# facebookresearch/ReAgent

Hardware: AMD Instinct MI355X
Metric: transitions/sec at batch=65536 state_dim=128; 1/2/4/8 MI355X scaling (higher is better)
Workload: dtype bf16; 1 GPU; Discrete DQN state_dim=128 |A|=16 3x512 MLP (BASELINE.json configs[1]; replay gather + normalize + 3 fwd + TD/Huber + bwd + Adam + soft update); batch=65536/GPU, 3x512 hidden; global_batch=65536, parallelism=dp1, launch=graph replay

## Files before the change

### profiles/microbench/fwd_phases.hip

```cpp
#include <hip/hip_runtime.h>
__device__ unsigned long long* g_stamps;
#define RG_STAMP(slot)                                                                                   \
  do {                                                                                                   \
    if ((threadIdx.x & 63) == 0)                                                                         \
      g_stamps[((long)blockIdx.x * (blockDim.x >> 6) + (threadIdx.x >> 6)) * 20 + (slot)] = __builtin_amdgcn_s_memtime(); \
  } while (0)
#include "../../reagent_amd/csrc/mlp_fused.hip"
namespace rg {
int x3_forward_launch(const rg_mlp_desc*, MlpArgs&, hipStream_t) { return RG_EINVAL; }
int x3_backward_launch(const rg_mlp_desc*, MlpArgs&, hipStream_t) { return RG_EINVAL; }
void grouped_bias_reduce_launch(const float*, const int*, int, int, float*, int, hipStream_t) {}
}
#include <cstdio>
#include <vector>

namespace rg {
template <int TN, int NW, int PITCH>
__global__ void RG_LAUNCH_BOUNDS(NW * 64, 1) fwd_some_save_kernel(MlpArgs saving, MlpArgs plain, int every) {
  if ((int)blockIdx.x & every) mlp_fwd_fused_body<TN, NW, PITCH, false>(saving);
  else mlp_fwd_fused_body<TN, NW, PITCH, false>(plain);
}
}

int main(int argc, char** argv) {
  using namespace rg;
  const int save = argc > 1 ? atoi(argv[1]) : 0;
  const int B = 65536, dims[5] = {128, 512, 512, 512, 16};
  MlpArgs a{};
  a.n_layers = 4; a.batch = B;
  for (int i = 0; i < 5; ++i) a.dims[i] = dims[i];
  for (int l = 0; l < 4; ++l) {
    a.acts[l] = l < 3 ? ACT_RELU : ACT_LINEAR;
    void* w; const size_t n = rg_wfrag_elems(dims[l + 1], dims[l]);
    hipMalloc(&w, n * 2); hipMemset(w, 0x3c, n * 2);
    a.wfrag[l] = (const bf16_t*)w;
    float* b; hipMalloc((void**)&b, dims[l + 1] * 4); hipMemset(b, 0, dims[l + 1] * 4);
    a.bias[l] = b;
    if (save) {
      void* f; hipMalloc(&f, rg_frag_elems(B, dims[l]) * 2); a.act_frag[l] = (bf16_t*)f;
      if (l >= 1) { void* sg; hipMalloc(&sg, rg_sign_bytes(B, dims[l])); a.act_sign[l] = (unsigned*)sg; }
    }
  }
  float *x, *out;
  hipMalloc((void**)&x, (size_t)B * 128 * 4); hipMemset(x, 0x3c, (size_t)B * 128 * 4);
  hipMalloc((void**)&out, (size_t)B * 16 * 4);
  a.x = x; a.ldx = 128; a.x_is_f32 = 1; a.out32 = out; a.ldo = 16; a.pitch = 520; a.save = save;
  const int n_wg = argc > 2 ? atoi(argv[2]) : B / 128, NPH = 20, NWV = FB_NW;
  unsigned long long* stamps;
  hipMalloc((void**)&stamps, (size_t)n_wg * NWV * NPH * 8);
  hipMemcpyToSymbol(HIP_SYMBOL(g_stamps), &stamps, sizeof(stamps));
  a.out_lds = argc > 3 ? atoi(argv[3]) : 0;
  const size_t lds = (size_t)128 * 520 * 2 + (a.out_lds ? 32 * 512 : 0);
  const int every = argc > 4 ? atoi(argv[4]) : 0;
  MlpArgs plain = a;
  plain.save = 0;
  hipFuncSetAttribute((const void*)mlp_fwd_fused_kernel<512 / (32 * FB_NW), FB_NW, 520>, hipFuncAttributeMaxDynamicSharedMemorySize, (int)lds);
  hipFuncSetAttribute((const void*)fwd_some_save_kernel<512 / (32 * FB_NW), FB_NW, 520>, hipFuncAttributeMaxDynamicSharedMemorySize, (int)lds);
  auto launch = [&] {
    if (every) fwd_some_save_kernel<512 / (32 * FB_NW), FB_NW, 520><<<n_wg, FB_NW * 64, lds>>>(a, plain, every);
    else mlp_fwd_fused_kernel<512 / (32 * FB_NW), FB_NW, 520><<<n_wg, FB_NW * 64, lds>>>(a);
  };
  hipEvent_t e0, e1; hipEventCreate(&e0); hipEventCreate(&e1);
  for (int w = 0; w < 3; ++w) launch();
  hipDeviceSynchronize();
  hipEventRecord(e0);
  for (int r = 0; r < 20; ++r) launch();
  hipEventRecord(e1); hipEventSynchronize(e1);
  float ms; hipEventElapsedTime(&ms, e0, e1);
  printf("forward NW=%d RING=%d save=%d: %.2f us/launch (stamps on), err=%d\n", FB_NW, MlpCfg<FB_NW>::RING, save, ms * 1e3 / 20, (int)hipGetLastError());
  std::vector<unsigned long long> h((size_t)n_wg * NWV * NPH);
  hipMemcpy(h.data(), stamps, h.size() * 8, hipMemcpyDeviceToHost);
  const char* names[NPH] = {"", "x tile load+barrier", "L0 mainloop(K=128)", "L0 pack", "L0 barrier wait", "L0 LDS store+barrier",
                            "L1 mainloop(K=512)", "L1 pack", "L1 barrier wait", "L1 LDS store+barrier",
                            "L2 mainloop(K=512)", "L2 pack", "L2 barrier wait", "L2 LDS store+barrier", "output layer", ""};
  double tot[NPH] = {0}, span = 0;
  int n_counted = 0;
  for (int g = 0; g < n_wg; ++g) {
    if (every && !(g & every)) continue;
    ++n_counted;
    for (int w = 0; w < NWV; ++w) {
      const unsigned long long* s = &h[((size_t)g * NWV + w) * NPH];
      for (int p = 1; p <= 14; ++p) tot[p] += (double)(s[p] - s[p - 1]);
      span += (double)(s[14] - s[0]);
    }
  }
  const double nw = (double)n_counted * NWV;
  if (every) printf("only workgroups with (index & %d) save: the tables below cover those %d\n", every, n_counted);
  printf("workgroups %d, shader clock %.3f GHz (ticks of one round / launch time)\n", n_wg, (span / nw) * ((n_wg + 255) / 256) / (ms * 1e6 / 20));
  printf("avg s_memtime ticks per wave: %.0f\n", span / nw);
  for (int p = 1; p <= 14; ++p) printf("  %-22s %9.0f ticks  %5.1f %%\n", names[p], tot[p] / nw, 100.0 * tot[p] / span);
  {
    double t[4] = {0, 0, 0, 0}, t19 = 0, n19 = 0;
    for (int g = 0; g < n_wg; ++g)
      for (int w = 0; w < NWV; ++w) {
        const unsigned long long* s = &h[((size_t)g * NWV + w) * NPH];
        if (!s[16] || (every && !(g & every))) continue;
        if (s[19]) { t19 += (double)(s[19] - s[18]); n19 += 1; }
        t[0] += (double)(s[16] - s[13]); t[1] += (double)(s[17] - s[16]); t[2] += (double)(s[18] - s[17]); t[3] += (double)(s[14] - s[18]);
      }
    printf("  storing waves: LDS sum %.0f ticks (of their sum + stores)\n", t19 / (n19 > 0 ? n19 : 1));
    printf("  output layer split: K loop %.0f | barrier wait %.0f | hand-off + barrier %.0f | sum + stores %.0f ticks\n", t[0] / nw, t[1] / nw, t[2] / nw, t[3] / nw);
  }
  printf("per-wave L1 main loop / barrier wait (ticks), averaged over workgroups:\n");
  for (int w = 0; w < NWV; ++w) {
    double ml = 0, bw = 0, ep = 0;
    for (int g = 0; g < n_wg; ++g) {
      const unsigned long long* s = &h[((size_t)g * NWV + w) * NPH];
      ml += (double)(s[6] - s[5]); bw += (double)(s[7] - s[6]); ep += (double)(s[8] - s[7]);
    }
    printf("  wave %d: mainloop %8.0f  pack %8.0f  wait %8.0f\n", w, ml / n_wg, bw / n_wg, ep / n_wg);
  }
  return 0;
}
```

### reagent_amd/csrc/mlp_fused.hip

```cpp

#include "rg_mlp_frag.h"
#include "rg_reduce.h"
#include "rg_dqn_head_row.h"

namespace rg {

constexpr int GROUPED_RING = 8;

template <int NW> struct MlpCfg {
  static constexpr int THREADS = NW * 64;
  static constexpr int RING = NW == 4 ? 8 : 2;
};

template <int NW>
__device__ __forceinline__ void grouped_whole_tile_out(bf16_t* act, int pitch, int KC, const bf16_t* wf_out, const float* b_out,
                                                                 int N, int NTo, int out_act, int lo, int hi, int row_base,
                                                                 const int* scatter, int batch, float* out32, long ldo) {
  const int tid = threadIdx.x, lane = tid & 63, wave = wave_uniform(tid >> 6), lr = lane & 31, lg = lane >> 5;
  const int P = NTo * 32 + 4, np = N >> 2;
  f32x16 acc4[4][1];
#pragma unroll
  for (int tm = 0; tm < 4; ++tm)
#pragma unroll
    for (int r = 0; r < 16; ++r) acc4[tm][0][r] = 0.f;
  const int col = wave * 32 + lr;
  float b = 0.f;
  if (wave < NTo) {
    if (b_out && col < N) b = b_out[col];
    wide_mainloop<1, GROUPED_RING>(act, pitch, KC, wf_out + (long)wave * KC * 512, 0, acc4, lane, k_rotation(blockIdx.x, wave, KC));
  }
  RG_STAMP(16);
  __syncthreads();
  RG_STAMP(17);
  float* stage = (float*)act;
  if (wave < NTo) {
#pragma unroll
    for (int tm = 0; tm < 4; ++tm) {
      float v[16];
#pragma unroll
      for (int r = 0; r < 16; ++r) v[r] = acc4[tm][0][r] + b;
      act_apply_n(v, out_act);
#pragma unroll
      for (int r = 0; r < 16; ++r) stage[(tm * 32 + (r & 3) + 8 * (r >> 2) + 4 * lg) * P + col] = v[r];
    }
  }
  __syncthreads();
  RG_STAMP(18);
  for (int rel = lo + wave; rel < hi; rel += NW) {
    int row = row_base + rel;
    if (scatter) row = scatter[row];
    if (row >= 0 && (scatter || row < batch) && lane < np)
      stream_store(*(const f32x4*)(stage + rel * P + lane * 4), (f32x4*)(out32 + (long)row * ldo + lane * 4));
  }
  RG_STAMP(19);
}

template <int TN, int NW, int PITCH, bool GROUPED, bool PAIR = false>
__device__ __forceinline__ void mlp_fwd_fused_body(const MlpArgs& a, const PairArgs* pp = nullptr, int pass = 0, bool on_state = false) {
  constexpr int THREADS = MlpCfg<NW>::THREADS, RING = MlpCfg<NW>::RING;
  static_assert(!PAIR || (!GROUPED && NW == 8), "the pair is the plain 8-wave kernel");
  const int save = PAIR ? (on_state ? 1 : 0) : a.save;
  RG_DYN_LDS(smem);
  bf16_t* act = (bf16_t*)smem;
  const int tid = PAIR ? opaque((int)threadIdx.x) : (int)threadIdx.x, lane = tid & 63, wave = wave_uniform(tid >> 6);
  const int lr = lane & 31, lg = lane >> 5;
  const int tile = GROUPED ? grouped_tile(blockIdx.x, (a.batch + FB_BM - 1) / FB_BM) : (int)blockIdx.x;
  if (GROUPED && tile * FB_BM >= round_up(a.batch, FB_BM)) return;
  const int row_base = tile * FB_BM;
  constexpr int pitch = PITCH;
  const int k0p = round_up(a.dims[0], 32);
  RG_STAMP(0);
  if constexpr (PAIR) {
    const PairIO& io = pp->io[on_state ? 1 : 0];
    const void* x = io.x;
    const long ldx = io.ldx;
    if (io.x_is_f32)
      load_tile_to_lds<float, THREADS>(act, pitch, (const float*)x, ldx, row_base, a.batch, a.dims[0], k0p, tid);
    else
      load_tile_to_lds<bf16_t, THREADS>(act, pitch, (const bf16_t*)x, ldx, row_base, a.batch, a.dims[0], k0p, tid);
  } else if (a.rowmap) {
    if (a.x_is_f32)
      load_tile_rows_mapped<float, THREADS>(act, pitch, (const float*)a.x, a.ldx, a.rowmap, row_base, a.dims[0], k0p, tid);
    else
      load_tile_rows_mapped<bf16_t, THREADS>(act, pitch, (const bf16_t*)a.x, a.ldx, a.rowmap, row_base, a.dims[0], k0p, tid);
  } else if (a.x2) {
    const int n2 = a.dims[0] - a.x_split;
    if (a.x_is_f32)
      load_tile_to_lds<float, THREADS>(act, pitch, (const float*)a.x, a.ldx, row_base, a.batch, a.x_split, a.x_split, tid, a.x_tile);
    else
      load_tile_to_lds<bf16_t, THREADS>(act, pitch, (const bf16_t*)a.x, a.ldx, row_base, a.batch, a.x_split, a.x_split, tid, a.x_tile);
    if (a.x2_is_f32)
      load_tile_to_lds<float, THREADS>(act + a.x_split, pitch, (const float*)a.x2, a.ldx2, row_base, a.batch, n2, k0p - a.x_split, tid);
    else
      load_tile_to_lds<bf16_t, THREADS>(act + a.x_split, pitch, (const bf16_t*)a.x2, a.ldx2, row_base, a.batch, n2, k0p - a.x_split, tid);
  } else if (a.x_is_f32)
    load_tile_to_lds<float, THREADS>(act, pitch, (const float*)a.x, a.ldx, row_base, a.batch, a.dims[0], k0p, tid);
  else
    load_tile_to_lds<bf16_t, THREADS>(act, pitch, (const bf16_t*)a.x, a.ldx, row_base, a.batch, a.dims[0], k0p, tid);
  __syncthreads();
  RG_STAMP(1);
  if (save == 1 && a.act_frag[0]) emit_frags_from_lds(act, pitch, k0p / 32, a.act_frag[0], tile * 4, wave, NW, lane);
  const bool out_lds = PAIR || (!GROUPED && a.out_lds);
  char* wo = (char*)(act + FB_BM * pitch);
  if (out_lds && pass == 0) out_lds_prefetch(a.wfrag[a.n_layers - 1], (a.dims[a.n_layers - 1] + 15) / 16, wo, wave, NW, lane);

  for (int l = 0; l < a.n_layers; ++l) {
    const int K = a.dims[l], N = a.dims[l + 1];
    const int KC = (K + 15) / 16;
    if (l < a.n_layers - 1) {
      f32x16 acc[4][TN];
#pragma unroll
      for (int tm = 0; tm < 4; ++tm)
#pragma unroll
        for (int tn = 0; tn < TN; ++tn)
#pragma unroll
          for (int r = 0; r < 16; ++r) acc[tm][tn][r] = 0.f;
      const long nt_stride = (long)KC * 512;
      wide_mainloop<TN, RING>(act, pitch, KC, a.wfrag[l] + (long)(wave * TN) * nt_stride, nt_stride, acc, lane,
                              k_rotation(blockIdx.x, wave, KC), wave / (NW / 2));
      RG_STAMP(2 + 4 * l);
      unsigned PK[4][TN][8];
      unsigned* sign_dst = save ? a.act_sign[l + 1] : nullptr;
      if constexpr (PAIR) {
        fwd_hidden_pack<TN, ACT_RELU>(acc, a.bias[l], save ? a.act_frag[l + 1] : nullptr, sign_dst, N / 32, tile * 4, wave, lane, PK);
      } else {
        RG_DISPATCH_ACT(a.acts[l], (fwd_hidden_pack<TN, A_>(acc, a.bias[l], fwd_save_dst(a, l),
                                                            sign_dst, N / 32, tile * 4, wave, lane, PK)));
      }
      RG_STAMP(3 + 4 * l);
      __syncthreads();
      RG_STAMP(4 + 4 * l);
      store_packed_tiles<TN>(act, pitch, PK, wave, lane);
      if (out_lds) RG_WAIT_VMCNT(0);
      __syncthreads();
      RG_STAMP(5 + 4 * l);
    } else {
      const int NTo = (N + 31) / 32;
      const int out_act = a.acts[l];
      const bool stream_out = N > 64;
      int seg_g = GROUPED ? a.tile_key[tile] : 0;
      RowSegment seg{0, 0, FB_BM};
      const int o_lane = GROUPED ? opaque(lane) : lane, o_tid = GROUPED ? opaque(tid) : tid;
      while (!GROUPED || next_segment(a.row_begin, a.n_groups, row_base, FB_BM, seg_g, seg)) {
        const int lane = o_lane, tid = o_tid, lr = lane & 31, lg = lane >> 5;
        const int grp = seg.grp;
        const bf16_t* wf_out = a.wfrag[l] + (GROUPED ? (long)grp * a.group_stride : 0);
        const float* b_out = a.bias[l] ? a.bias[l] + (GROUPED ? (long)grp * N : 0) : nullptr;
        const int tm0 = GROUPED ? seg.lo >> 5 : 0, tm1 = GROUPED ? (seg.hi + 31) >> 5 : 4;
        const float b_tile0 = (b_out && lr < N) ? b_out[lr] : 0.f;
        auto store_tile = [&](const f32x16& acc, int tm, int nt) {
          const int col = nt * 32 + lr;
          if (col < N) {
            const float b = nt == 0 ? b_tile0 : (b_out ? b_out[col] : 0.f);
            float ov[16];
#pragma unroll
            for (int r = 0; r < 16; ++r) ov[r] = acc[r] + b;
            act_apply_n(ov, out_act);
#pragma unroll
            for (int r = 0; r < 16; ++r) {
              const int rel = tm * 32 + (r & 3) + 8 * (r >> 2) + 4 * lg;
              if (GROUPED && (rel < seg.lo || rel >= seg.hi)) continue;
              int row = row_base + rel;
              if (a.out_scatter) row = a.rowmap[row];
              if (row >= 0 && (a.out_scatter || row < a.batch)) {
                const float o = ov[r];
                if (stream_out) stream_store(o, a.out32 + (long)row * a.ldo + col);
                else a.out32[(long)row * a.ldo + col] = o;
              }
            }
          }
        };
        f32x4 h_m4, h_qt4, h_ac4;
        float h_rew = 0.f, h_nt = 0.f, h_ge = 0.f;
        int h_b = 0;
        bool h_live = false;
        if constexpr (PAIR) {
          if (pass == 1) {
            const int it = wave * 64 + opaque(lane), row = row_base + (it >> 2);
            h_live = row < a.batch;
            h_b = h_live ? row : a.batch - 1;
            const long o = (long)h_b * 16 + (it & 3) * 4;
            h_m4 = *(const f32x4*)(pp->next_mask + o);
            h_qt4 = *(const f32x4*)(pp->qn_target + o);
            h_ac4 = *(const f32x4*)(pp->action + o);
            h_rew = pp->reward[h_b];
            h_nt = pp->not_terminal[h_b];
            if (pp->gamma_exponent) h_ge = pp->gamma_exponent[h_b];
          }
        }
        if (PAIR || (!GROUPED && NTo == 1 && NW == 8 && KC >= 8)) {
          const int tm = wave & 3, half = wave >> 2, kc_mid = (KC / 2 + 3) / 4 * 4;
          f32x16 acc = out_lds ? tile_kloop_ldsb(act, pitch, wo, tm, lane, half ? kc_mid : 0, half ? KC : kc_mid)
                               : tile_kloop(act, pitch, KC, wf_out, tm, 0, lane, half ? kc_mid : 0, half ? KC : kc_mid);
          RG_STAMP(16);
          __syncthreads();
          RG_STAMP(17);
          const int o_ln = opaque(lane), o_lr = o_ln & 31, o_lg = o_ln >> 5;
          const bool aligned16 = (reinterpret_cast<uintptr_t>(a.out32) & 15) == 0;
          const bool dense_run = a.ldo == N && row_base + FB_BM <= a.batch;
          const bool rowstore = PAIR || (!a.out_scatter && aligned16 && (dense_run || ((N & 3) == 0 && (a.ldo & 3) == 0)));
          if (rowstore) {
            float* outs = (float*)act + half * (FB_BM * 32);
            float* bias_s = (float*)act + 2 * (FB_BM * 32);
            if (o_lr < N) {
#pragma unroll
              for (int r = 0; r < 16; ++r) outs[(tm * 32 + (r & 3) + 8 * (r >> 2) + 4 * o_lg) * N + o_lr] = acc[r];
              if (wave == 0 && o_lg == 0) bias_s[o_lr] = b_tile0;
            }
            __syncthreads();
            RG_STAMP(18);
            RG_STAMP(19);
            const float* lo_ = (const float*)act;
            const float* hi_ = lo_ + FB_BM * 32;
            if constexpr (PAIR) {
              const int it = wave * 64 + o_ln, rel = it >> 2, c4 = it & 3, row = row_base + rel;
              const f32x4 l4 = *(const f32x4*)(lo_ + it * 4), h4 = *(const f32x4*)(hi_ + it * 4);
              const f32x4 b4 = *(const f32x4*)(bias_s + c4 * 4);
              float o[4];
#pragma unroll
              for (int e = 0; e < 4; ++e) o[e] = (l4[e] + h4[e]) + b4[e];
              act_apply_n(o, out_act);
              const f32x4 mine = f32x4{o[0], o[1], o[2], o[3]};
              if (row < a.batch) *(f32x4*)(pp->io[on_state ? 1 : 0].out + (long)row * 16 + c4 * 4) = mine;
              f32x4* park = (f32x4*)(wo + (size_t)KC * 512);
              if (pass == 0) {
                park[it] = mine;
              } else {
                const f32x4 other = park[it];
                const f32x4 q4 = on_state ? mine : other, qon4 = on_state ? other : mine;
                const float loss = dqn_head_lanes_row<4>(h_m4, h_qt4, pp->double_q ? qon4 : h_qt4, h_ac4, q4, c4, h_b, h_live, h_rew,
                                                         pp->reward_boosts, h_nt, pp->gamma, pp->gamma_exponent != nullptr, h_ge,
                                                         a.batch, pp->double_q, pp->loss_type, pp->dq, pp->next_q, pp->next_idx,
                                                         pp->q_sel);
                const float ws = dqn_head_wave_sum(loss);
                if (o_ln == 0) pp->wave_sums[tile * NW + wave] = ws;
              }
            } else if (dense_run) {
              float* dst = a.out32 + (long)row_base * N;
              for (int it = wave * 64 + o_ln; it < (FB_BM * N) >> 2; it += THREADS) {
                const f32x4 l4 = *(const f32x4*)(lo_ + it * 4), h4 = *(const f32x4*)(hi_ + it * 4);
                float o[4];
#pragma unroll
                for (int e = 0; e < 4; ++e) o[e] = (l4[e] + h4[e]) + bias_s[(it * 4 + e) % N];
                act_apply_n(o, out_act);
                *(f32x4*)(dst + it * 4) = f32x4{o[0], o[1], o[2], o[3]};
              }
            }
            const int np = N >> 2;
            for (int it = wave * 64 + o_ln; !PAIR && !dense_run && it < FB_BM * np; it += THREADS) {
              const int rel = it / np, c4 = it - rel * np;
              const int row = row_base + rel;
              if (row < a.batch) {
                const f32x4 l4 = *(const f32x4*)(lo_ + rel * N + c4 * 4), h4 = *(const f32x4*)(hi_ + rel * N + c4 * 4);
                const f32x4 b4 = *(const f32x4*)(bias_s + c4 * 4);
                float o[4];
#pragma unroll
                for (int e = 0; e < 4; ++e) o[e] = (l4[e] + h4[e]) + b4[e];
                act_apply_n(o, out_act);
                *(f32x4*)(a.out32 + (long)row * a.ldo + c4 * 4) = f32x4{o[0], o[1], o[2], o[3]};
              }
            }
          } else {
            float* hand = (float*)act + (tm * 64 + lane) * 16;
            if (half) {
#pragma unroll
              for (int r = 0; r < 16; r += 4) *(f32x4*)(hand + r) = f32x4{acc[r], acc[r + 1], acc[r + 2], acc[r + 3]};
            }
            __syncthreads();
            RG_STAMP(18);
            if (!half) {
#pragma unroll
              for (int r = 0; r < 16; r += 4) {
                const f32x4 o = *(const f32x4*)(hand + r);
                acc[r] += o[0]; acc[r + 1] += o[1]; acc[r + 2] += o[2]; acc[r + 3] += o[3];
              }
              RG_STAMP(19);
              store_tile(acc, tm, 0);
            }
          }
        } else if (GROUPED && NTo <= NW && a.stage_out) {
          const int P = NTo * 32 + 4;
          const int np = N >> 2;
          bool last_segment = false;
          if ((size_t)FB_BM * P * sizeof(float) <= (size_t)FB_BM * pitch * sizeof(bf16_t)) {
            int g2 = seg_g;
            RowSegment s2;
            last_segment = !next_segment(a.row_begin, a.n_groups, row_base, FB_BM, g2, s2);
          }
          if (last_segment) {
            grouped_whole_tile_out<NW>(act, pitch, KC, wf_out, b_out, N, NTo, out_act, seg.lo, seg.hi, row_base, a.out_scatter ? a.rowmap : nullptr,
                                       a.batch, a.out32, a.ldo);
            break;
          }
          float* stage = (float*)(act + FB_BM * pitch);
          for (int tm = tm0; tm < tm1; ++tm) {
            if (wave < NTo) {
              const f32x16 acc = tile_kloop(act, pitch, KC, wf_out, tm, wave, lane);
              const int col = wave * 32 + lr;
              const float b = (b_out && col < N) ? b_out[col] : 0.f;
              float v[16];
#pragma unroll
              for (int r = 0; r < 16; ++r) v[r] = acc[r] + b;
              act_apply_n(v, out_act);
#pragma unroll
              for (int r = 0; r < 16; ++r) stage[((r & 3) + 8 * (r >> 2) + 4 * lg) * P + col] = v[r];
            }
            __syncthreads();
            for (int it = tid; it < 32 * np; it += THREADS) {
              const int r = it / np, c4 = it - r * np;
              const int rel = tm * 32 + r;
              if (rel < seg.lo || rel >= seg.hi) continue;
              int row = row_base + rel;
              if (a.out_scatter) row = a.rowmap[row];
              if (row >= 0 && (a.out_scatter || row < a.batch))
                stream_store(*(const f32x4*)(stage + r * P + c4 * 4), (f32x4*)(a.out32 + (long)row * a.ldo + c4 * 4));
            }
            __syncthreads();
          }
        } else {
          for (int t = wave; t < 4 * NTo; t += NW) {
            const int tm = t & 3, nt = t >> 2;
            if (tm < tm0 || tm >= tm1) continue;
            store_tile(tile_kloop(act, pitch, KC, wf_out, tm, nt, lane), tm, nt);
          }
        }
        if (!GROUPED) break;
      }
      RG_STAMP(2 + 4 * l);
    }
  }
}

#ifndef RG_PAIR_ORDER_SHIFT
#define RG_PAIR_ORDER_SHIFT 0
#endif
template <int TN, int NW, int PITCH>
__global__ void RG_LAUNCH_BOUNDS(NW * 64, 1) mlp_fwd_pair_kernel(MlpArgs a, PairArgs p) {
  const bool state_first = (((int)blockIdx.x >> RG_PAIR_ORDER_SHIFT) & 1) != 0;
  mlp_fwd_fused_body<TN, NW, PITCH, false, true>(a, &p, 0, state_first);
  __syncthreads();
  mlp_fwd_fused_body<TN, NW, PITCH, false, true>(a, &p, 1, !state_first);
}

template <int TN, int NW, int PITCH>
__global__ void RG_LAUNCH_BOUNDS(NW * 64, 1) mlp_fwd_fused_kernel(MlpArgs a) {
  mlp_fwd_fused_body<TN, NW, PITCH, false>(a);
}
template <int TN, int NW, int PITCH>
__global__ void RG_LAUNCH_BOUNDS(NW * 64, 1) mlp_fwd_grouped_kernel(MlpArgs a) {
  mlp_fwd_fused_body<TN, NW, PITCH, true>(a);
}

template <int TN, int NW, int PITCH, bool DX_ONLY, bool GROUPED = false>
__device__ __forceinline__ void mlp_bwd_fused_body(const MlpArgs& a) {
  constexpr int THREADS = MlpCfg<NW>::THREADS, RING = MlpCfg<NW>::RING;
  RG_DYN_LDS(smem);
  bf16_t* act = (bf16_t*)smem;
  const int tid = threadIdx.x, lane = tid & 63, wave = wave_uniform(tid >> 6);
  const int lr = lane & 31, lg = lane >> 5;
  const int tile = GROUPED ? grouped_tile(blockIdx.x, (a.batch + FB_BM - 1) / FB_BM) : (int)blockIdx.x;
  if (tile * FB_BM >= round_up(a.batch, FB_BM)) return;
  const int row_base = tile * FB_BM;
  constexpr int pitch = PITCH;
  const int L = a.n_layers;
  const int nop = round_up(a.dims[L], 32);
  RG_BSTAMP(0);
  auto request_signs = [&](int l, unsigned (&sg)[2 * TN]) {
    if (a.act_sign[l] != nullptr) {
      const u32x2* sp = (const u32x2*)(a.act_sign[l] + sign_offset(tile, wave, lane, TN, a.dims[l]));
#pragma unroll
      for (int i = 0; i < TN; ++i) {
        const u32x2 t = sp[i];
        sg[2 * i] = t[0];
        sg[2 * i + 1] = t[1];
      }
    } else {
#pragma unroll
      for (int i = 0; i < 2 * TN; ++i) sg[i] = 0u;
    }
  };
  unsigned sg_first[2 * TN];
  if (L >= 2) request_signs(L - 1, sg_first);
  const bool first_one_chunk = !GROUPED && L >= 2 && a.dims[L] <= 16;
  u16x8 w_first[TN];
  if (first_one_chunk) {
    const bf16_t* wl = a.wfrag[L - 1] + (long)(wave * TN) * 512 + lane * 8;
#pragma unroll
    for (int tn = 0; tn < TN; ++tn) w_first[tn] = *(const u16x8*)(wl + tn * 512);
  }
  load_tile_to_lds<float, THREADS>(act, pitch, a.dout32, a.lddo, row_base, a.batch, a.dims[L], nop, tid);
  __syncthreads();
  RG_BSTAMP(1);
  if (!GROUPED) {
    if (!DX_ONLY) emit_frags_from_lds(act, pitch, nop / 32, a.dz_frag[L - 1], tile * 4, wave, NW, lane);
    if (a.db_part[L - 1] && tid < a.dims[L]) {
      float s = 0.f;
      for (int r = 0; r < FB_BM; ++r) s += bf16_to_f32(act[r * pitch + tid]);
      a.db_part[L - 1][(long)tile * a.dims[L] + tid] = s;
    }
  }
  RG_BSTAMP(2);

  for (int l = L - 1; l >= 1; --l) {
    const int K = a.dims[l + 1], N = a.dims[l];
    const int KC = (K + 15) / 16;
    f32x16 acc[4][TN];
#pragma unroll
    for (int tm = 0; tm < 4; ++tm)
#pragma unroll
      for (int tn = 0; tn < TN; ++tn)
#pragma unroll
        for (int r = 0; r < 16; ++r) acc[tm][tn][r] = 0.f;
    const long nt_stride = (long)KC * 512;
    unsigned sg[2 * TN];
    const bool use_sign = a.act_sign[l] != nullptr;
    if (l == L - 1) {
#pragma unroll
      for (int i = 0; i < 2 * TN; ++i) sg[i] = sg_first[i];
    } else {
      request_signs(l, sg);
    }
    const bool grouped_layer = GROUPED && l == L - 1;
    bf16_t* cp = act + masked_copy_offset<PITCH>(FB_BM * PITCH);
    int seg_g = grouped_layer ? a.tile_key[tile] : 0;
    RowSegment seg{0, 0, FB_BM};
    bool more = grouped_layer ? next_segment(a.row_begin, a.n_groups, row_base, FB_BM, seg_g, seg) : true;
    auto segment_side = [&]() -> const bf16_t* {
      const bool whole = seg.lo == 0 && seg.hi == FB_BM;
      if (!whole) {
        copy_rows_masked<THREADS, FB_BM>(act, cp, pitch, nop, seg.lo, seg.hi, tid);
        __syncthreads();
      }
      const bf16_t* src = whole ? act : cp;
      emit_frags_from_lds(src, pitch, nop / 32, a.dz_frag[L - 1], tile * 4 + seg.grp, wave, NW, lane, seg.lo >> 5,
                          (seg.hi + 31) >> 5);
      if (a.db_part[L - 1] && tid < a.dims[L]) {
        float s = 0.f;
        for (int r = seg.lo; r < seg.hi; ++r) s += bf16_to_f32(act[r * pitch + tid]);
        a.db_part[L - 1][(long)(tile + seg.grp) * a.dims[L] + tid] = s;
      }
      return src;
    };
    if (more) {
      const bf16_t* src = act;
      if (grouped_layer) src = segment_side();
      const bf16_t* wl = a.wfrag[l] + (grouped_layer ? (long)seg.grp * a.group_stride : 0);
      if (first_one_chunk && l == L - 1) {
        const bf16_t* arow = src + lr * pitch + lg * 8;
        u16x8 af[4];
#pragma unroll
        for (int tm = 0; tm < 4; ++tm) af[tm] = *(const u16x8*)(arow + tm * 32 * pitch);
#pragma unroll
        for (int tm = 0; tm < 4; ++tm)
#pragma unroll
          for (int tn = 0; tn < TN; ++tn) acc[tm][tn] = mfma_main(af[tm], w_first[tn], acc[tm][tn]);
      } else {
        wide_mainloop<TN, RING>(src, pitch, KC, wl + (long)(wave * TN) * nt_stride, nt_stride, acc, lane,
                                k_rotation(blockIdx.x, wave, KC), wave / (NW / 2));
      }
    }
    if (grouped_layer) {
      while (more && next_segment(a.row_begin, a.n_groups, row_base, FB_BM, seg_g, seg)) {
        __syncthreads();
        const bf16_t* src = segment_side();
        segment_accumulate<4, TN>(src, pitch, KC, a.wfrag[l] + (long)seg.grp * a.group_stride + (long)(wave * TN) * nt_stride,
                                  nt_stride, acc, lane);
      }
    }
    float* dbp = a.db_part[l - 1] ? a.db_part[l - 1] + (long)tile * N : nullptr;
    RG_BSTAMP(3 + 4 * (L - 1 - l));
    unsigned PK[4][TN][8];
    if (use_sign) {
      RG_DISPATCH_ACT(a.acts[l - 1], (bwd_hidden_pack<TN, A_, true, !DX_ONLY>(acc, a.act_frag[l], sg, a.dz_frag[l - 1], dbp,
                                                                             N / 32, tile * 4, wave, lane, PK)));
    } else {
      RG_DISPATCH_ACT(a.acts[l - 1], (bwd_hidden_pack<TN, A_, false, !DX_ONLY>(acc, a.act_frag[l], sg, a.dz_frag[l - 1], dbp,
                                                                              N / 32, tile * 4, wave, lane, PK)));
    }
    RG_BSTAMP(4 + 4 * (L - 1 - l));
    __syncthreads();
    RG_BSTAMP(5 + 4 * (L - 1 - l));
    store_packed_tiles<TN>(act, pitch, PK, wave, lane);
    __syncthreads();
    RG_BSTAMP(6 + 4 * (L - 1 - l));
  }
  if (a.dx32) {
    const int K = a.dims[1], N = a.dims[0];
    const int KC = (K + 15) / 16, NTi = (N + 31) / 32, nt0 = a.dx_col0 / 32;
    for (int t = wave; t < 4 * (NTi - nt0); t += NW) {
      const int tm = t & 3, nt = nt0 + (t >> 2);
      const f32x16 acc = tile_kloop(act, pitch, KC, a.wfrag[0], tm, nt, lane);
      const int col = nt * 32 + lr;
      if (col < N) {
#pragma unroll
// ... 213 lines not shown
```

### reagent_amd/csrc/rg_mlp_frag.h

```cpp
#pragma once
#include "rg_gemm.h"
#include "rg_optim.h"
#include <type_traits>
#include "../../include/reagent_hip.h"

#ifndef RG_STAMP
#define RG_STAMP(slot)
#endif
#ifndef RG_BSTAMP
#define RG_BSTAMP(slot)
#endif
#ifndef RG_PHASE_INIT
#define RG_PHASE_INIT()
#define RG_PHASE(i)
#define RG_PHASE_FLUSH()
#endif

namespace rg {

constexpr int FB_BM = 128;
constexpr int WG_THREADS = 512;
constexpr int FB_NW = 8;
constexpr int FB_MAXL = RG_MLP_MAX_LAYERS;

// ... 5 lines not shown
    const char* e = getenv("RG_X3_DZ_PLANES");
    const int n = e ? atoi(e) : RG_X3_DZ_PLANES;
    return n == 1 ? 1 : 2;
  }();
  return v;
}

struct MlpArgs {
  int n_layers, batch;
  int dims[FB_MAXL + 1];
  int acts[FB_MAXL];
  const bf16_t* wfrag[FB_MAXL];
  const float* bias[FB_MAXL];
  bf16_t* act_frag[FB_MAXL + 1];
  bf16_t* dz_frag[FB_MAXL];
  unsigned* act_sign[FB_MAXL];
  float* db_part[FB_MAXL];
  const void* x;
  long ldx;
  const void* x2;
  long ldx2;
  int x_split;
  int x_tile;
  int dx_col0;
  const int* rowmap;
  const int* tile_key;
  const int* row_begin;
  int n_groups;
  long group_stride;
  int out_scatter;
  int stage_out;
  int out_lds;
  int x_is_f32, x2_is_f32;
  float* out32;
  long ldo;
  const float* dout32;
  long lddo;
  float* dx32;
  long lddx;
  int pitch;
  int save;
  long wfrag_lo[FB_MAXL];
  long act_lo[FB_MAXL + 1];
  long dz_lo[FB_MAXL];
};

struct PairIO {
  const void* x;
  long ldx;
  float* out;
  int x_is_f32, pad_;
};
struct PairArgs {
  PairIO io[2];
  const float *qn_target, *action, *next_mask, *reward, *reward_boosts, *not_terminal, *gamma_exponent;
  float gamma;
  int double_q, loss_type;
  float* dq;
  float* wave_sums;
  float* next_q;
  int64_t* next_idx;
  float* q_sel;
};

__device__ __forceinline__ int round_up(int x, int m) { return (x + m - 1) / m * m; }

template <int ACT> __device__ __forceinline__ float act_t(float z) { return act_apply(z, ACT); }

template <int ACT> __device__ __forceinline__ float act_grad_t(float h) { return act_grad_from_output(h, ACT); }
#define RG_DISPATCH_ACT(act, ...)                                                   \
  switch (act) {                                                                    \
    case ACT_RELU: { constexpr int A_ = ACT_RELU; __VA_ARGS__; } break;             \
    case ACT_LEAKY_RELU: { constexpr int A_ = ACT_LEAKY_RELU; __VA_ARGS__; } break; \
    case ACT_TANH: { constexpr int A_ = ACT_TANH; __VA_ARGS__; } break;             \
    case ACT_SIGMOID: { constexpr int A_ = ACT_SIGMOID; __VA_ARGS__; } break;       \
    case ACT_SOFTPLUS: { constexpr int A_ = ACT_SOFTPLUS; __VA_ARGS__; } break;     \
    default: { constexpr int A_ = ACT_LINEAR; __VA_ARGS__; } break;                 \
  }

__device__ __forceinline__ long frag_offset(int mb, int nt, int NT, int h, int lane) {
  return ((((long)mb * NT + nt) * 2 + h) * 64 + lane) * 8;
}
__device__ __forceinline__ int frag_row(int h, int e, int lg) {
  const int r = 8 * h + e;
  return (r & 3) + 8 * (r >> 2) + 4 * lg;
}

template <typename T, int THREADS>
__device__ __forceinline__ void load_tile_to_lds(bf16_t* act, int pitch, const T* src, long ld, int row_base,
                                                 int nrows, int ncols, int ncols_pad, int tid, int xt = 1) {
  const int cpr = ncols_pad / 8;
  const int total = FB_BM * cpr;
  const bool vec = ((ld % 8) == 0) && ((((uintptr_t)src) & 15) == 0);
  if (vec && (ncols & 7) == 0 && ncols > 0) {
    constexpr int U = 4;
    const int kmax = ncols - 8;
    for (int c0 = tid; c0 < total; c0 += THREADS * U) {
      f32x4 raw[U][sizeof(T) == 4 ? 2 : 1];
#pragma unroll
      for (int u = 0; u < U; ++u) {
        const int cu = c0 + u * THREADS, c = cu < total ? cu : total - 1;
        const int gr = row_base + c / cpr, grow = gr < nrows ? gr : nrows - 1;
        const int kk = (c % cpr) * 8;
        const T* p = src + (long)(xt > 1 ? grow / xt : grow) * ld + (kk < kmax ? kk : kmax);
        raw[u][0] = *(const f32x4*)p;
        if (sizeof(T) == 4) raw[u][sizeof(T) == 4 ? 1 : 0] = *(const f32x4*)(p + 4);
      }
#pragma unroll
      for (int u = 0; u < U; ++u) {
        const int c = c0 + u * THREADS;
        if (c >= total) break;
        const int r = c / cpr, k0 = (c % cpr) * 8;
        u16x8 v;
        if (sizeof(T) == 4) {
#pragma unroll
          for (int e = 0; e < 4; ++e) {
            v[e] = f32_to_bf16(raw[u][0][e]);
            v[4 + e] = f32_to_bf16(raw[u][sizeof(T) == 4 ? 1 : 0][e]);
          }
        } else {
          v = __builtin_bit_cast(u16x8, raw[u][0]);
        }
        if (row_base + r >= nrows || k0 >= ncols) v = u16x8{0, 0, 0, 0, 0, 0, 0, 0};
        *(u16x8*)&act[r * pitch + k0] = v;
      }
    }
    return;
  }
  for (int c = tid; c < total; c += THREADS) {
    const int r = c / cpr, k0 = (c % cpr) * 8;
    const int grow = row_base + r;
    u16x8 v = {0, 0, 0, 0, 0, 0, 0, 0};
    if (grow < nrows && k0 < ncols) {
      const T* p = src + (long)(xt > 1 ? grow / xt : grow) * ld + k0;
      if (sizeof(T) == 2 && vec && k0 + 8 <= ncols) {
        v = *(const u16x8*)p;
      } else if (sizeof(T) == 4 && vec && k0 + 8 <= ncols) {
        const f32x4 a = *(const f32x4*)p, b = *(const f32x4*)(p + 4);
#pragma unroll
        for (int e = 0; e < 4; ++e) {
          v[e] = cvt_out<bf16_t>(a[e]);
          v[4 + e] = cvt_out<bf16_t>(b[e]);
        }
      } else {
#pragma unroll
        for (int e = 0; e < 8; ++e)
          if (k0 + e < ncols) v[e] = cvt_out<bf16_t>(cvt_in(p[e]));
      }
    }
    *(u16x8*)&act[r * pitch + k0] = v;
  }
}

template <typename T, int THREADS>
__device__ __forceinline__ void load_tile_rows_mapped(bf16_t* act, int pitch, const T* src, long ld, const int* rowmap,
                                                      int row_base, int ncols, int ncols_pad, int tid) {
  const int cpr = ncols_pad / 8;
  const int total = FB_BM * cpr;
  const bool vec = ((ld % 8) == 0) && ((((uintptr_t)src) & 15) == 0);
  for (int c = tid; c < total; c += THREADS) {
    const int r = c / cpr, k0 = (c % cpr) * 8;
    const int grow = rowmap[row_base + r];
    u16x8 v = {0, 0, 0, 0, 0, 0, 0, 0};
    if (grow >= 0 && k0 < ncols) {
      const T* p = src + (long)grow * ld + k0;
      if (sizeof(T) == 2 && vec && k0 + 8 <= ncols) {
        v = *(const u16x8*)p;
      } else if (sizeof(T) == 4 && vec && k0 + 8 <= ncols) {
        const f32x4 a = *(const f32x4*)p, b = *(const f32x4*)(p + 4);
#pragma unroll
        for (int e = 0; e < 4; ++e) {
          v[e] = cvt_out<bf16_t>(a[e]);
          v[4 + e] = cvt_out<bf16_t>(b[e]);
        }
      } else {
#pragma unroll
        for (int e = 0; e < 8; ++e)
          if (k0 + e < ncols) v[e] = cvt_out<bf16_t>(cvt_in(p[e]));
      }
    }
    *(u16x8*)&act[r * pitch + k0] = v;
  }
}

__device__ __forceinline__ void emit_frags_from_lds(const bf16_t* act, int pitch, int ntiles, bf16_t* dst,
                                                    int mb_base, int wave, int n_waves, int lane, int mbl0 = 0, int mbl1 = 4) {
  const int lr = lane & 31, lg = lane >> 5;
  const int total = (mbl1 - mbl0) * ntiles * 2;
  for (int f = wave; f < total; f += n_waves) {
    const int h = f & 1, nt = (f >> 1) % ntiles, mbl = mbl0 + (f >> 1) / ntiles;
    u16x8 v;
#pragma unroll
    for (int e = 0; e < 8; ++e) v[e] = act[(mbl * 32 + frag_row(h, e, lg)) * pitch + nt * 32 + lr];
    *(u16x8*)(dst + frag_offset(mb_base + mbl, nt, ntiles, h, lane)) = v;
  }
}

__device__ __forceinline__ void pack_tile(const float (&v)[16], unsigned (&P)[8]) {
#pragma unroll
  for (int i = 0; i < 8; ++i) P[i] = pack_bf16x2(v[2 * i], v[2 * i + 1]);
}

__device__ __forceinline__ void store_packed_to_lds(bf16_t* act, int pitch, int row0_tile, int col, int lane,
                                                    const unsigned (&P)[8]) {
  const int lg = lane >> 5, odd = lane & 1;
  const unsigned sel = odd ? 0x03020706u : 0x05040100u;
  bf16_t* base = act + (row0_tile + 4 * lg + odd) * pitch + (col & ~1);
#pragma unroll
  for (int i = 0; i < 8; ++i) {
    const int r = 2 * i;
    const unsigned other = swap_adjacent_lanes(P[i]);
    const unsigned word = perm_bytes(other, P[i], sel);
    *(unsigned*)(base + ((r & 3) + 8 * (r >> 2)) * pitch) = word;
  }
}

typedef __attribute__((ext_vector_type(4))) unsigned u32x4;
__device__ __forceinline__ void store_packed_frags(bf16_t* dst, int mb, int nt, int NT, int lane,
                                                   const unsigned (&P)[8]) {
#pragma unroll
  for (int h = 0; h < 2; ++h) {
    const u32x4 v = u32x4{P[4 * h], P[4 * h + 1], P[4 * h + 2], P[4 * h + 3]};
    stream_store(v, (u32x4*)(dst + frag_offset(mb, nt, NT, h, lane)));
  }
}

template <bool NONNEG>
__device__ __forceinline__ unsigned positive_bits(const float (&v)[16]) {
  unsigned bits = 0u;
#pragma unroll
  for (int r = 15; r >= 0; --r) {
    if (NONNEG) bits = (bits << 1) | ((0u - __builtin_bit_cast(unsigned, v[r])) >> 31);
    else bits = (bits << 1) | (v[r] > 0.f ? 1u : 0u);
  }
  return bits;
}

__device__ __forceinline__ int grouped_tile(int block, int n_tiles) {
  const int per = (n_tiles + 7) >> 3;
  return (block & 7) * per + (block >> 3);
}

struct RowSegment {
  int grp, lo, hi;
};
__device__ __forceinline__ bool next_segment(const int* row_begin, int n_groups, int row_base, int rows, int& g, RowSegment& s) {
  while (g >= 0 && g < n_groups) {
    const int b = row_begin[g], e = row_begin[g + 1];
    if (b >= row_base + rows) return false;
    const int lo = b > row_base ? b : row_base, hi = e < row_base + rows ? e : row_base + rows;
    const int grp = g++;
    if (hi > lo) {
      s.grp = grp;
      s.lo = lo - row_base;
      s.hi = hi - row_base;
      return true;
    }
  }
  return false;
}

template <int THREADS, int ROWS>
__device__ __forceinline__ void copy_rows_masked(const bf16_t* src, bf16_t* dst, int pitch, int ncols, int lo, int hi, int tid) {
  const int cpr = ncols >> 3;
  for (int c = tid; c < ROWS * cpr; c += THREADS) {
    const int r = c / cpr, k = (c - r * cpr) * 8;
    u16x8 v = *(const u16x8*)(src + r * pitch + k);
    if (r < lo || r >= hi) v = u16x8{0, 0, 0, 0, 0, 0, 0, 0};
    *(u16x8*)(dst + r * pitch + k) = v;
  }
}
template <int PITCH> __device__ __forceinline__ constexpr int masked_copy_offset(int tile_elems) {
  return PITCH >= 2 * 256 + 8 ? 256 : tile_elems;
}

__device__ __forceinline__ int k_rotation(int wg, int wave, int KC) { return (wg * 5 + wave * 11) % KC; }

__device__ __forceinline__ f32x16 mfma_main(u16x8 a, u16x8 b, f32x16 c) { return mfma_32x32x16_bf16(a, b, c); }

template <int TN, int RING>
__device__ __forceinline__ void wide_mainloop(const bf16_t* act, int pitch, int KC, const bf16_t* wf_wave,
                                              long nt_stride, f32x16 (&acc)[4][TN], int lane, int rot,
                                              int prio_phase = 0) {
  static_assert(RING >= 2 && RING % 2 == 0, "the A double buffer alternates with the ring slot parity");
  const int lr = lane & 31, lg = lane >> 5;
  auto kx = [&](int kc) { const int k = kc + rot; return k >= KC ? k - KC : k; };
  const bf16_t* arow = act + lr * pitch + lg * 8;
  const int tm_stride = 32 * pitch;
  u16x8 a[2][4], b[RING][TN];
  auto loadB = [&](u16x8 (&bf)[TN], int kc) {
    const bf16_t* chunk = wf_wave + (long)kx(kc) * 512;
#pragma unroll
    for (int tn = 0; tn < TN; ++tn) bf[tn] = *(const u16x8*)(chunk + tn * nt_stride + lane * 8);
  };
  auto loadA = [&](u16x8 (&af)[4], int kc) {
    const int off = kx(kc) * 16;
#pragma unroll
    for (int tm = 0; tm < 4; ++tm) af[tm] = *(const u16x8*)(arow + tm * tm_stride + off);
  };
  auto mma = [&](const u16x8 (&af)[4], const u16x8 (&bf)[TN]) {
#pragma unroll
    for (int tm = 0; tm < 4; ++tm)
#pragma unroll
      for (int tn = 0; tn < TN; ++tn) acc[tm][tn] = mfma_main(af[tm], bf[tn], acc[tm][tn]);
  };
  if (KC % RING == 0) {
// ... 345 lines not shown
```

Measured before the change: 134.5 million transitions/s.

## Prefetch second pass input tile into registers during first pass output layer

In the paired forward kernel, the first pass now issues global loads for the other input's 128-row tile into registers (HeldTile) at the start of the output layer. The second pass then writes those held values into LDS instead of loading the tile from global memory, hiding the load latency behind the output-layer compute. It also hoists the output-layer bias load once per kernel. The cost is extra VGPRs (32 floats per thread) and a forced vmcnt(0) wait before the prefetch, which could hurt occupancy or stall. The microbench gains a pair mode with per-pass stamps.

```diff
diff --git a/profiles/microbench/fwd_phases.hip b/profiles/microbench/fwd_phases.hip
--- a/profiles/microbench/fwd_phases.hip
+++ b/profiles/microbench/fwd_phases.hip
@@ -1,9 +1,10 @@
 #include <hip/hip_runtime.h>
 __device__ unsigned long long* g_stamps;
+namespace rg { constexpr int pass = 0; }
 #define RG_STAMP(slot)                                                                                   \
   do {                                                                                                   \
     if ((threadIdx.x & 63) == 0)                                                                         \
-      g_stamps[((long)blockIdx.x * (blockDim.x >> 6) + (threadIdx.x >> 6)) * 20 + (slot)] = __builtin_amdgcn_s_memtime(); \
+      g_stamps[((long)blockIdx.x * (blockDim.x >> 6) + (threadIdx.x >> 6)) * 40 + 20 * pass + (slot)] = __builtin_amdgcn_s_memtime(); \
   } while (0)
 #include "../../reagent_amd/csrc/mlp_fused.hip"
 namespace rg {
@@ -12,6 +13,7 @@
 void grouped_bias_reduce_launch(const float*, const int*, int, int, float*, int, hipStream_t) {}
 }
 #include <cstdio>
+#include <cstring>
 #include <vector>
 
 namespace rg {
@@ -22,8 +24,88 @@
 }
 }
 
+static int pair_main(bool f32_rows) {
+  using namespace rg;
+  const int B = 65536, dims[5] = {128, 512, 512, 512, 16}, n_wg = B / 128, NPH = 40, NWV = FB_NW;
+  auto dmalloc = [](size_t bytes, int fill) { void* p; hipMalloc(&p, bytes); hipMemset(p, fill, bytes); return p; };
+  auto ones = [&](size_t n) {
+    std::vector<float> h(n, 1.f);
+    void* p = dmalloc(n * 4, 0);
+    hipMemcpy(p, h.data(), n * 4, hipMemcpyHostToDevice);
+    return (float*)p;
+  };
+  MlpArgs a{};
+  a.n_layers = 4; a.batch = B;
+  for (int i = 0; i < 5; ++i) a.dims[i] = dims[i];
+  for (int l = 0; l < 4; ++l) {
+    a.acts[l] = l < 3 ? ACT_RELU : ACT_LINEAR;
+    a.wfrag[l] = (const bf16_t*)dmalloc(rg_wfrag_elems(dims[l + 1], dims[l]) * 2, 0x3c);
+    a.bias[l] = (const float*)dmalloc(dims[l + 1] * 4, 0);
+    a.act_frag[l] = (bf16_t*)dmalloc(rg_frag_elems(B, dims[l]) * 2, 0);
+    if (l >= 1) a.act_sign[l] = (unsigned*)dmalloc(rg_sign_bytes(B, dims[l]), 0);
+  }
+  a.ldo = 16; a.pitch = 520; a.out_lds = 1;
+  PairArgs p{};
+  const size_t esz = f32_rows ? 4 : 2;
+  for (int i = 0; i < 2; ++i) p.io[i] = PairIO{dmalloc((size_t)B * 128 * esz, 0x3c), 128, (float*)dmalloc((size_t)B * 64, 0), f32_rows, 0};
+  p.qn_target = (const float*)dmalloc((size_t)B * 64, 0x3c);
+  p.action = (const float*)dmalloc((size_t)B * 64, 0);
+  p.next_mask = ones((size_t)B * 16);
+  p.reward = (const float*)dmalloc((size_t)B * 4, 0x3c);
+  p.not_terminal = ones(B);
+  p.gamma = 0.99f; p.double_q = 1; p.loss_type = RG_LOSS_HUBER;
+  p.dq = (float*)dmalloc((size_t)B * 64, 0);
+  p.wave_sums = (float*)dmalloc((size_t)n_wg * NWV * 4, 0);
+  p.next_q = (float*)dmalloc((size_t)B * 4, 0);
+  p.next_idx = (int64_t*)dmalloc((size_t)B * 8, 0);
+  p.q_sel = (float*)dmalloc((size_t)B * 4, 0);
+  unsigned long long* stamps = (unsigned long long*)dmalloc((size_t)n_wg * NWV * NPH * 8, 0);
+  hipMemcpyToSymbol(HIP_SYMBOL(g_stamps), &stamps, sizeof(stamps));
+  const size_t lds = (size_t)128 * 520 * 2 + 32 * 512 + 128 * 16 * 4;
+  hipFuncSetAttribute((const void*)mlp_fwd_pair_kernel<2, FB_NW, 520>, hipFuncAttributeMaxDynamicSharedMemorySize, (int)lds);
+  auto launch = [&] { mlp_fwd_pair_kernel<2, FB_NW, 520><<<n_wg, FB_NW * 64, lds>>>(a, p); };
+  hipEvent_t e0, e1; hipEventCreate(&e0); hipEventCreate(&e1);
+  for (int w = 0; w < 3; ++w) launch();
+  hipDeviceSynchronize();
+  hipEventRecord(e0);
+  for (int r = 0; r < 20; ++r) launch();
+  hipEventRecord(e1); hipEventSynchronize(e1);
+  float ms; hipEventElapsedTime(&ms, e0, e1);
+  printf("pair forward, %s rows: %.2f us/launch (stamps on), err=%d\n", f32_rows ? "fp32" : "bf16", ms * 1e3 / 20, (int)hipGetLastError());
+  std::vector<unsigned long long> h((size_t)n_wg * NWV * NPH);
+  hipMemcpy(h.data(), stamps, h.size() * 8, hipMemcpyDeviceToHost);
+  const char* names[15] = {"", "x tile -> LDS+barrier", "L0 mainloop(K=128)", "L0 pack", "L0 barrier wait", "L0 LDS store+barrier",
+                           "L1 mainloop(K=512)", "L1 pack", "L1 barrier wait", "L1 LDS store+barrier",
+                           "L2 mainloop(K=512)", "L2 pack", "L2 barrier wait", "L2 LDS store+barrier", "output layer"};
+  for (int order = 0; order < 2; ++order) {
+    double tot[2][15] = {}, between = 0, span = 0, kloop[2] = {0, 0};
+    int n = 0;
+    for (int g = 0; g < n_wg; ++g) {
+      if (((g >> RG_PAIR_ORDER_SHIFT) & 1) != order) continue;
+      ++n;
+      for (int w = 0; w < NWV; ++w) {
+        const unsigned long long* s = &h[((size_t)g * NWV + w) * NPH];
+        for (int ps = 0; ps < 2; ++ps) {
+          for (int ph = 1; ph <= 14; ++ph) tot[ps][ph] += (double)(s[20 * ps + ph] - s[20 * ps + ph - 1]);
+          kloop[ps] += (double)(s[20 * ps + 16] - s[20 * ps + 13]);
+        }
+        between += (double)(s[20] - s[14]);
+        span += (double)(s[34] - s[0]);
+      }
+    }
+    const double nw = (double)n * NWV;
+    printf("order %s: %d workgroups, avg ticks per wave %.0f (between the passes %.0f)\n",
+           order ? "(state: saving, next_state)" : "(next_state, state: saving)", n, span / nw, between / nw);
+    printf("  %-24s %12s %12s\n", "", "first pass", "second pass");
+    for (int ph = 1; ph <= 14; ++ph) printf("  %-24s %12.0f %12.0f\n", names[ph], tot[0][ph] / nw, tot[1][ph] / nw);
+    printf("  %-24s %12.0f %12.0f\n", "(output layer's K loop)", kloop[0] / nw, kloop[1] / nw);
+  }
+  return 0;
+}
+
 int main(int argc, char** argv) {
   using namespace rg;
+  if (argc > 1 && !strcmp(argv[1], "pair")) return pair_main(argc > 2 && !strcmp(argv[2], "f32"));
   const int save = argc > 1 ? atoi(argv[1]) : 0;
   const int B = 65536, dims[5] = {128, 512, 512, 512, 16};
   MlpArgs a{};
@@ -45,7 +127,7 @@
   hipMalloc((void**)&x, (size_t)B * 128 * 4); hipMemset(x, 0x3c, (size_t)B * 128 * 4);
   hipMalloc((void**)&out, (size_t)B * 16 * 4);
   a.x = x; a.ldx = 128; a.x_is_f32 = 1; a.out32 = out; a.ldo = 16; a.pitch = 520; a.save = save;
-  const int n_wg = argc > 2 ? atoi(argv[2]) : B / 128, NPH = 20, NWV = FB_NW;
+  const int n_wg = argc > 2 ? atoi(argv[2]) : B / 128, NPH = 40, NWV = FB_NW;
   unsigned long long* stamps;
   hipMalloc((void**)&stamps, (size_t)n_wg * NWV * NPH * 8);
   hipMemcpyToSymbol(HIP_SYMBOL(g_stamps), &stamps, sizeof(stamps));
diff --git a/reagent_amd/csrc/mlp_fused.hip b/reagent_amd/csrc/mlp_fused.hip
--- a/reagent_amd/csrc/mlp_fused.hip
+++ b/reagent_amd/csrc/mlp_fused.hip
@@ -56,7 +56,8 @@
 }
 
 template <int TN, int NW, int PITCH, bool GROUPED, bool PAIR = false>
-__device__ __forceinline__ void mlp_fwd_fused_body(const MlpArgs& a, const PairArgs* pp = nullptr, int pass = 0, bool on_state = false) {
+__device__ __forceinline__ void mlp_fwd_fused_body(const MlpArgs& a, const PairArgs* pp = nullptr, int pass = 0, bool on_state = false,
+                                                   HeldTile* held = nullptr) {
   constexpr int THREADS = MlpCfg<NW>::THREADS, RING = MlpCfg<NW>::RING;
   static_assert(!PAIR || (!GROUPED && NW == 8), "the pair is the plain 8-wave kernel");
   const int save = PAIR ? (on_state ? 1 : 0) : a.save;
@@ -74,7 +75,10 @@
     const PairIO& io = pp->io[on_state ? 1 : 0];
     const void* x = io.x;
     const long ldx = io.ldx;
-    if (io.x_is_f32)
+    if (pass == 1 && tile_holdable(x, ldx, a.dims[0], k0p, THREADS)) {
+      if (io.x_is_f32) tile_commit<float, THREADS>(act, pitch, *held, row_base, a.batch, a.dims[0], k0p, tid);
+      else tile_commit<bf16_t, THREADS>(act, pitch, *held, row_base, a.batch, a.dims[0], k0p, tid);
+    } else if (io.x_is_f32)
       load_tile_to_lds<float, THREADS>(act, pitch, (const float*)x, ldx, row_base, a.batch, a.dims[0], k0p, tid);
     else
       load_tile_to_lds<bf16_t, THREADS>(act, pitch, (const bf16_t*)x, ldx, row_base, a.batch, a.dims[0], k0p, tid);
@@ -103,6 +107,11 @@
   const bool out_lds = PAIR || (!GROUPED && a.out_lds);
   char* wo = (char*)(act + FB_BM * pitch);
   if (out_lds && pass == 0) out_lds_prefetch(a.wfrag[a.n_layers - 1], (a.dims[a.n_layers - 1] + 15) / 16, wo, wave, NW, lane);
+  float b_pair = 0.f;
+  if constexpr (PAIR) {
+    const float* bo = a.bias[a.n_layers - 1];
+    if (bo && lr < 16) b_pair = bo[lr];
+  }
 
   for (int l = 0; l < a.n_layers; ++l) {
     const int K = a.dims[l], N = a.dims[l + 1];
@@ -147,7 +156,7 @@
         const bf16_t* wf_out = a.wfrag[l] + (GROUPED ? (long)grp * a.group_stride : 0);
         const float* b_out = a.bias[l] ? a.bias[l] + (GROUPED ? (long)grp * N : 0) : nullptr;
         const int tm0 = GROUPED ? seg.lo >> 5 : 0, tm1 = GROUPED ? (seg.hi + 31) >> 5 : 4;
-        const float b_tile0 = (b_out && lr < N) ? b_out[lr] : 0.f;
+        const float b_tile0 = PAIR ? b_pair : (b_out && lr < N) ? b_out[lr] : 0.f;
         auto store_tile = [&](const f32x16& acc, int tm, int nt) {
           const int col = nt * 32 + lr;
           if (col < N) {
@@ -175,6 +184,16 @@
         int h_b = 0;
         bool h_live = false;
         if constexpr (PAIR) {
+          if (pass == 0) {
+            const PairIO& nx = pp->io[on_state ? 0 : 1];
+            const int d0 = a.dims[0], d0p = round_up(d0, 32);
+            wait_vmcnt0_known();
+            if (tile_holdable(nx.x, nx.ldx, d0, d0p, THREADS)) {
+              const int it = wave * 64 + opaque(lane);
+              if (nx.x_is_f32) tile_request<float, THREADS>(*held, (const float*)nx.x, nx.ldx, row_base, a.batch, d0, d0p, it);
+              else tile_request<bf16_t, THREADS>(*held, (const bf16_t*)nx.x, nx.ldx, row_base, a.batch, d0, d0p, it);
+            }
+          }
           if (pass == 1) {
             const int it = wave * 64 + opaque(lane), row = row_base + (it >> 2);
             h_live = row < a.batch;
@@ -337,9 +356,10 @@
 template <int TN, int NW, int PITCH>
 __global__ void RG_LAUNCH_BOUNDS(NW * 64, 1) mlp_fwd_pair_kernel(MlpArgs a, PairArgs p) {
   const bool state_first = (((int)blockIdx.x >> RG_PAIR_ORDER_SHIFT) & 1) != 0;
-  mlp_fwd_fused_body<TN, NW, PITCH, false, true>(a, &p, 0, state_first);
+  HeldTile held;
+  mlp_fwd_fused_body<TN, NW, PITCH, false, true>(a, &p, 0, state_first, &held);
   __syncthreads();
-  mlp_fwd_fused_body<TN, NW, PITCH, false, true>(a, &p, 1, !state_first);
+  mlp_fwd_fused_body<TN, NW, PITCH, false, true>(a, &p, 1, !state_first, &held);
 }
 
 template <int TN, int NW, int PITCH>
diff --git a/reagent_amd/csrc/rg_mlp_frag.h b/reagent_amd/csrc/rg_mlp_frag.h
--- a/reagent_amd/csrc/rg_mlp_frag.h
+++ b/reagent_amd/csrc/rg_mlp_frag.h
@@ -181,6 +181,56 @@
   }
 }
 
+__device__ __forceinline__ void wait_vmcnt0_known() {
+#if defined(__HIP_DEVICE_COMPILE__)
+  __builtin_amdgcn_s_waitcnt(0x0F70);
+#endif
+}
+struct HeldTile {
+  f32x4 raw[4][2];
+};
+__device__ __forceinline__ bool tile_holdable(const void* src, long ld, int ncols, int ncols_pad, int threads) {
+  const bool vec = ((ld % 8) == 0) && ((((uintptr_t)src) & 15) == 0);
+  return vec && (ncols & 7) == 0 && ncols > 0 && FB_BM * (ncols_pad / 8) <= threads * 4;
+}
+template <typename T, int THREADS>
+__device__ __forceinline__ void tile_request(HeldTile& t, const T* src, long ld, int row_base, int nrows, int ncols,
+                                             int ncols_pad, int tid) {
+  const int cpr = ncols_pad / 8, total = FB_BM * cpr, kmax = ncols - 8;
+#pragma unroll
+  for (int u = 0; u < 4; ++u) {
+    const int cu = tid + u * THREADS, c = cu < total ? cu : total - 1;
+    const int gr = row_base + c / cpr, grow = gr < nrows ? gr : nrows - 1;
+    const int kk = (c % cpr) * 8;
+    const T* p = src + (long)grow * ld + (kk < kmax ? kk : kmax);
+    t.raw[u][0] = *(const f32x4*)p;
+    if (sizeof(T) == 4) t.raw[u][1] = *(const f32x4*)(p + 4);
+  }
+}
+template <typename T, int THREADS>
+__device__ __forceinline__ void tile_commit(bf16_t* act, int pitch, const HeldTile& t, int row_base, int nrows, int ncols,
+                                            int ncols_pad, int tid) {
+  const int cpr = ncols_pad / 8, total = FB_BM * cpr;
+#pragma unroll
+  for (int u = 0; u < 4; ++u) {
+    const int c = tid + u * THREADS;
+    if (c >= total) break;
+    const int r = c / cpr, k0 = (c % cpr) * 8;
+    u16x8 v;
+    if (sizeof(T) == 4) {
+#pragma unroll
+      for (int e = 0; e < 4; ++e) {
+        v[e] = f32_to_bf16(t.raw[u][0][e]);
+        v[4 + e] = f32_to_bf16(t.raw[u][1][e]);
+      }
+    } else {
+      v = __builtin_bit_cast(u16x8, t.raw[u][0]);
+    }
+    if (row_base + r >= nrows || k0 >= ncols) v = u16x8{0, 0, 0, 0, 0, 0, 0, 0};
+    *(u16x8*)&act[r * pitch + k0] = v;
+  }
+}
+
 template <typename T, int THREADS>
 __device__ __forceinline__ void load_tile_rows_mapped(bf16_t* act, int pitch, const T* src, long ld, const int* rowmap,
                                                       int row_base, int ncols, int ncols_pad, int tid) {
```

Result: no change. 134.9 million transitions/s, median of 3 (+0.3%).
